# tencent-ailab/pika

Hardware: NVIDIA H100
Metric: utterances/sec RNN-T train step (T=1000,U=150,V=6k) (higher is better)
Workload: dtype bf16

## Files before the change

### include/pika_b200.h

```cpp
#ifndef PIKA_B200_H
#define PIKA_B200_H
#include <stdint.h>

#ifdef __cplusplus
extern "C" {
#endif

#define PK_F32 0
#define PK_BF16 1

const char* pk_last_error(void);
int pk_version(void);
long long pk_launch_count(void);

#define PK_GEMM_MAX_PAIRS 9
#define PK_SEL_ZERO 0
#define PK_SEL_ZB0 1
#define PK_SEL_ZB1 2
#define PK_SEL_KZ 3
#define PK_ACT_NONE 0
#define PK_ACT_RELU 1
#define PK_AUX_NONE 0
#define PK_AUX_ADD 1
#define PK_AUX_MASK_NZ 2
// ... 144 lines not shown
                           const void* dout, long long ld_dout, const float* lse, float* dsum_ws, void* dq, void* dk, void* dv,
                           long long ld_dqkv, int B, int T, int heads, int dh, float alpha, float drop_p, const uint32_t* keep_bits,
                           int chunk_len, int chunk_off, int left_chunks, void* stream);
int pk_attention_chunk_admits_all(int T, int chunk_len, int chunk_off, int left_chunks);
long long pk_colstats_ws_floats(int C);
int pk_bn_fwd(const void* x, void* y, int dtype, long long rows, int C, const float* w, const float* b, float eps,
              int train, float momentum, float* run_mean, float* run_var, float* mean, float* rstd, float* stats_ws,
              void* stream);
int pk_bn_bwd(const void* dy, const void* x, void* dx, int dtype, long long rows, int C, const float* w,
              const float* mean, const float* rstd, int train, int relu_mask, float* dw, float* db, float* ws ,
              void* stream);
int pk_colsum(const void* x, int dtype, long long rows, int C, float* out, float* ws, void* stream);
int pk_layernorm_fwd(const void* x, void* y, int dtype, long long rows, int C, const float* w, const float* b, float eps,
                     float* mean, float* rstd, void* stream);
int pk_layernorm_bwd(const void* dy, const void* x, void* dx, int dtype, long long rows, int C, const float* w,
                     const float* mean, const float* rstd, float* dw, float* db, void* stream);
int pk_softmax_fwd(const float* S, long long ld_s, void* P, void* Pd, int dtype, long long ld_p, long long rows, int n,
                   float drop_p, uint32_t seed, void* stream);
int pk_softmax_masked_fwd(const float* S, long long ld_s, void* P, void* Pd, int dtype, long long ld_p, long long rows, int n,
                          int q_len, int heads, int causal, const uint8_t* key_pad, float drop_p, uint32_t seed, void* stream);
int pk_softmax_chunk_fwd(const float* S, long long ld_s, void* P, void* Pd, int dtype, long long ld_p, long long rows, int n,
                         int chunk_len, int chunk_off, int left_chunks, float drop_p, uint32_t seed, void* stream);
int pk_softmax_bwd(const float* dPd, long long ld_d, const void* P, long long ld_p, void* dS, int dtype, long long rows,
                   int n, float drop_p, uint32_t seed, void* stream);
#define PK_RELPOS_MAX 1024
int pk_softmax_masked_relpos_fwd(const float* S, long long ld_s, const float* QR, long long ld_r, void* P, void* Pd, int dtype,
                                 long long ld_p, long long rows, int n, int q_len, int heads, int causal, const uint8_t* key_pad,
                                 int max_rel, float* Pb, float drop_p, uint32_t seed, void* stream);
int pk_softmax_relpos_bwd(const float* dPd, long long ld_d, const float* G, long long ld_r, const void* P, long long ld_p, void* dS,
                          int dtype, long long rows, int n, int q_len, int heads, int max_rel, float* dSb, float drop_p,
                          uint32_t seed, void* stream);
int pk_dropout(const void* x, void* y, int dtype, long long n, float p, uint32_t seed, void* stream);
int pk_mask_nz(const void* dy, const void* y, void* dx, int dtype, long long n, float scale, void* stream);
int pk_add(const void* a, const void* b, void* o, int dtype, long long n, void* stream);
int pk_log_softmax(const void* x, int dtype, long long ld, float* y, long long rows, int n, float scale, void* stream);
int pk_joint_gate_fwd(const void* ex, const void* py, void* h, int dtype, int B, int T, int U1, int H, int ld_h, void* stream);
int pk_joint_gate_bwd(const void* ex, const void* py, const void* dh, const int* dh_map, void* dex, void* dpy, int dtype, int B, int T,
                      int U1, int H, void* stream);
int pk_lstm_cell_fwd(const float* gx, long long ld_gx, const float* gh, long long ld_gh, const float* c_prev, float* c_out,
                     void* h_out, int dtype, long long ld_h, float* gates_save, int B, int H, void* stream);
int pk_lstm_cell_bwd(const void* dh_out, long long ld_dho, const float* dh_rec, const float* dc_next, const float* gates,
                     const float* c, const float* c_prev, void* dgates, int dtype, float* dc_prev, int B, int H, void* stream);
int pk_embedding_fwd(const long long* idx, const float* table, int E, void* out, int dtype, int ld_out, long long n, void* stream);
int pk_embedding_bwd(const long long* idx, const void* dout, int dtype, int ld, int E, float* dtable, long long n,
                     long long padding_idx, void* stream);

int pk_absmax(const float* x, long long n, float* out, int* nan_flag, void* stream);
int pk_sgd_nesterov_clip(float* p, const float* g, float* buf, long long n, float lr, float momentum, float max_norm,
                         const float* absmax, const int* nan_flag, int first, void* stream);
int pk_bmuf_delta(const float* glob, const float* local, float* delta, long long n, void* stream);
int pk_bmuf_update(float* glob, float* local, float* delta_prev, const float* delta_sum, long long n, int world,
                   float block_momentum, float block_lr, void* stream);
int pk_adam_clip(float* p, const float* g, float* exp_avg, float* exp_avg_sq, float* p_out2, long long n, double lr,
                 double beta1, double beta2, double eps, double bias_correction1, double bias_correction2_sqrt,
                 float max_norm, const float* absmax, const int* nan_flag, void* stream);
int pk_bmuf_adam_update(float* glob, float* local, float* delta_prev, float* exp_avg_g, float* exp_avg_sq_g, float* msg,
                        long long n, int world, double block_momentum, double block_lr, double beta1_tau, double beta1_rho,
                        double beta2_tau, double beta2_rho, void* stream);

long long pk_frontend_workspace_bytes(int B, int n_max, int t_max, int n_mel, int D);
int pk_frontend_fwd(const short* pcm, long long ld_pcm, const int* n_samples, const float* rate, const int* new_len,
                    const float* target_db, const int* n_frames, int B, int n_max, int t_max, int n_mel, int lctx,
                    int rctx, int stride, const float* window, const float* twiddle, const float* mel_w, const int* mel_lo,
                    const int* mel_hi, int frame_len, int frame_shift, int log2_nfft, int snip_edges, int remove_dc,
                    float preemph, int cmn, const float* offset, const float* scale, int f0, int fs,
                    int t0, int ts, void* out, int out_dtype, short* wave_i16_out, void* workspace,
                    long long workspace_bytes, int* err_flag, float dither, unsigned int dither_seed, void* stream);
int pk_fbank(const float* wave, long long ld_wave, const int* n_samples, const int* n_frames, int B, int t_max, int n_mel,
             const float* window, const float* twiddle, const float* mel_w, const int* mel_lo, const int* mel_hi, int frame_len,
             int frame_shift, int log2_nfft, int snip_edges, int remove_dc, float preemph, float* feats, float dither,
             unsigned int dither_seed, void* stream);

long long pk_frontend_noise_rir_workspace_bytes(int B, int n_max, int t_max, int n_mel, int D, int rir_max_len);
int pk_frontend_fwd_noise_rir(const short* pcm, long long ld_pcm, const int* n_samples, const float* rate, const int* new_len,
                              const float* target_db, const int* n_frames, int B, int n_max, int t_max, int n_mel, int lctx,
                              int rctx, int stride, const float* window, const float* twiddle, const float* mel_w,
                              const int* mel_lo, const int* mel_hi, int frame_len, int frame_shift, int log2_nfft, int snip_edges,
                              int remove_dc, float preemph, int cmn, const float* offset, const float* scale, int f0, int fs,
                              int t0, int ts, void* out, int out_dtype, short* wave_i16_out, void* workspace,
                              long long workspace_bytes, int* err_flag, float dither, unsigned int dither_seed, void* stream,
                              const short* noise, const int* noise_idx, const long long* noise_off, const double* snr,
                              const double* noise_rms_db, const short* rir, const long long* rir_off, const int* rir_len,
                              const int* rir_idx, int rir_max_len);

int pk_mfcc(const float* wave, long long ld_wave, const int* n_samples, const int* n_frames, int B, int t_max, int n_mel,
            const float* window, const float* twiddle, const float* mel_w, const int* mel_lo, const int* mel_hi, int frame_len,
            int frame_shift, int log2_nfft, int snip_edges, int remove_dc, float preemph, float* feats, float dither,
            unsigned int dither_seed, void* stream, const float* dct, int num_ceps, int use_energy, int raw_energy,
            float energy_floor, int htk_compat);
int pk_frontend_fwd_mfcc(const short* pcm, long long ld_pcm, const int* n_samples, const float* rate, const int* new_len,
                         const float* target_db, const int* n_frames, int B, int n_max, int t_max, int n_mel, int lctx,
                         int rctx, int stride, const float* window, const float* twiddle, const float* mel_w,
                         const int* mel_lo, const int* mel_hi, int frame_len, int frame_shift, int log2_nfft, int snip_edges,
                         int remove_dc, float preemph, int cmn, const float* offset, const float* scale, int f0, int fs,
                         int t0, int ts, void* out, int out_dtype, short* wave_i16_out, void* workspace,
                         long long workspace_bytes, int* err_flag, float dither, unsigned int dither_seed, void* stream,
                         const short* noise, const int* noise_idx, const long long* noise_off, const double* snr,
                         const double* noise_rms_db, const short* rir, const long long* rir_off, const int* rir_len,
                         const int* rir_idx, int rir_max_len, const float* dct, int num_ceps, int use_energy,
                         int raw_energy, float energy_floor, int htk_compat);

long long pk_conv_same_f64_workspace_bytes(int B, int n_max, int m_max);
int pk_conv_same_f64(const double* x, long long ld_x, const int* n_len, const double* h, long long ld_h, const int* m_len, int B,
                     int n_max, int m_max, double* y, long long ld_y, void* workspace, long long workspace_bytes, void* stream);

int pk_beam_prepare(const int* next_ys, const int* step_ctx, int* t_idx, const void* enc, int dtype, int Tenc, int H, void* enc_hid,
                    const float* embed, int E, void* x_emb, int ld_x, int K, int blk, int rows, void* stream);
int pk_beam_lstm_cell(const float* gates, const int* next_ys, const int* step_ctx, int blk, void* h, int dtype, float* c, int rows, int H,
                      void* stream);
int pk_beam_step_end(int* step_ctx, const int* not_done, int max_steps, void* stream);
int pk_beam_gate(const float* a, void* h, int dtype, int rows, int H, void* stream);
int pk_row_lse(const void* x, int dtype, long long ld, float* lse, long long rows, int n, float scale, void* stream);
int pk_beam_advance(const float* logits, int ldv, const float* row_lse, float sm_scale, const int* t_idx, const int* num_frames, const int* max_len, float* scores,
                    int* next_ys, int* prev_ks, int* hyp_tok, int* hyp_len, float* fin_score, int* fin_step, int* fin_k,
                    int* fin_count, int* eos_top, int* done, int* not_done_total, int B, int K, int V, int L, int cap,
                    const int* step_ctx, int blk, int n_best, int beam_prune, void* stream);
int pk_beam_reorder(const int* prev_ks, const int* step_ctx, const void* h_in, const float* c_in, const int* t_in, void* h_out, float* c_out,
                    int* t_out, int dtype, int K, int H, int layers, int rows, void* stream);
typedef struct {
    const int* arc_off;
    const int* arc_ilabel;
    const double* arc_weight;
    const int* arc_next;
    const double* finals;
    int backoff_id, n_disambig;
    int disambig_ids[4];
} pk_lm_fst;
int pk_beam_advance_lm(const float* logits, int ldv, const float* row_lse, float sm_scale, const int* t_idx, const int* num_frames, const int* max_len, float* scores,
                       int* next_ys, int* prev_ks, int* hyp_tok, int* hyp_len, float* fin_score, int* fin_step, int* fin_k,
                       int* fin_count, int* eos_top, int* done, int* not_done_total, int B, int K, int V, int L, int cap,
                       const int* step_ctx, int blk, int n_best, int beam_prune, const pk_lm_fst* fst, double lm_scale, double nonblk_reward,
                       int* set_state, double* set_cost, int* set_n, float* lm_scores, int max_states, int* err_flag, void* stream);

typedef struct {
    const int* next_ys;
    const int* step_ctx;
    const int* hyp_tok;
    const int* hyp_len;
    int* slot;
    void* pool;
    long long n_entries;
    int blk, rows, S1, layers, D, dtype, init;
} pk_beam_xf_state;
int pk_beam_xf_taps(const pk_beam_xf_state* st, int layer, const float* embed, int E, const void* x_cur, void* taps, int ldc, void* stream);
int pk_beam_xf_attn(const pk_beam_xf_state* st, int layer, const void* qkv, int heads, const float* rel, int max_rel, void* out, void* stream);
int pk_beam_xf_select(const pk_beam_xf_state* st, const void* x, void* h, int H, void* stream);
int pk_beam_xf_slots(const pk_beam_xf_state* st, const int* prev_ks, int K, void* stream);

long long pk_lstm_seq_workspace_bytes(int H);
int pk_lstm_seq_fwd_ex(const float* gx, const void* w_hh_bf16, void* out, int out_dtype, int ldo, float* gates_save, float* cs,
                       const int* lens, int B, int U, int H, int n_dir, int reverse, void* ws, void* stream);
int pk_lstm_seq_bwd_ex(const void* dout, int dtype, int ldo, const float* gates_save, const float* cs, const void* w_hh_bf16,
                       void* dG_bf16, const int* lens, int B, int U, int H, int n_dir, int reverse, void* ws, void* stream);

int pk_gather_rows(const void* src, const int* idx, void* dst, int dtype, long long rows, int C, void* stream);
int pk_scatter_add_rows(const void* src, const int* idx, float* dst, int dtype, long long rows, int C, void* stream);
int pk_ce_grad(const void* z, int dtype, long long ld, const int* tok, const float* coef, float scale, void* dz,
               long long rows, int n, void* stream);

#ifdef __cplusplus
}
#endif
#endif
```

### pika_b200/csrc/lstm_seq.cu

```cuda
#include <cooperative_groups.h>

#include "../../include/pika_b200.h"
#include "common.cuh"

namespace pk {
void count_launch();

constexpr int LS_HJ = 8;
constexpr int LS_MB = 32;
constexpr int LS_THREADS = 256;
constexpr int LS_PAD = 8;

PK_DEVICE void mma_bf16_16816(float (&c)[4], uint32_t a0, uint32_t a1, uint32_t a2, uint32_t a3, uint32_t b0, uint32_t b1) {
    asm volatile(
        "mma.sync.aligned.m16n8k16.row.col.f32.bf16.bf16.f32 {%0,%1,%2,%3}, {%4,%5,%6,%7}, {%8,%9}, {%0,%1,%2,%3};"
        : "+f"(c[0]), "+f"(c[1]), "+f"(c[2]), "+f"(c[3])
        : "r"(a0), "r"(a1), "r"(a2), "r"(a3), "r"(b0), "r"(b1));
}
PK_DEVICE uint4 ldcg16(const void* p) {
    uint4 r;
    asm volatile("ld.global.cg.v4.u32 {%0,%1,%2,%3}, [%4];" : "=r"(r.x), "=r"(r.y), "=r"(r.z), "=r"(r.w) : "l"(p));
    return r;
}
PK_DEVICE void bulk_g2s(void* smem_dst, const void* gsrc, uint32_t bytes, uint64_t* bar) {
    asm volatile("cp.async.bulk.shared::cluster.global.mbarrier::complete_tx::bytes [%0], [%1], %2, [%3];" ::"r"(smem_u32(smem_dst)),
                 "l"(gsrc), "r"(bytes), "r"(smem_u32(bar))
                 : "memory");
}
PK_DEVICE void bulk_g2s_mc(void* smem_dst, const void* gsrc, uint32_t bytes, uint64_t* bar, uint16_t mask) {
    asm volatile("cp.async.bulk.shared::cluster.global.mbarrier::complete_tx::bytes.multicast::cluster [%0], [%1], %2, [%3], %4;" ::"r"(
                     smem_u32(smem_dst)),
                 "l"(gsrc), "r"(bytes), "r"(smem_u32(bar)), "h"(mask)
                 : "memory");
}
PK_DEVICE void fence_proxy_async_all() { asm volatile("fence.proxy.async;" ::: "memory"); }

PK_DEVICE void grid_barrier(unsigned int* counter, unsigned int step_index, unsigned int nct) {
    const unsigned int target = nct * step_index;
    __syncthreads();
    if (threadIdx.x == 0) {
        asm volatile("red.release.gpu.global.add.u32 [%0], 1;" ::"l"(counter) : "memory");
        unsigned int seen;
        do {
            asm volatile("ld.acquire.gpu.global.u32 %0, [%1];" : "=r"(seen) : "l"(counter) : "memory");
        } while (seen < target);
    }
    __syncthreads();
}
PK_DEVICE float sigm(float x) { return 1.f / (1.f + __expf(-x)); }

PK_DEVICE void load_lens(const int* lens, int B, int U, int* len_s, int* steps_s) {
    if (threadIdx.x < 32) {
        int L = 0;
        if ((int)threadIdx.x < B) L = lens ? min(max(lens[threadIdx.x], 0), U) : U;
        len_s[threadIdx.x] = L;
        int m = L;
#pragma unroll
        for (int o = 16; o > 0; o >>= 1) m = max(m, __shfl_xor_sync(0xffffffffu, m, o));
        if (threadIdx.x == 0) *steps_s = m;
    }
}

struct LsDir {
    int d;
    bool rev;
    int j0;
    unsigned nct;
};
PK_DEVICE LsDir ls_dir(int H, int reverse) {
    LsDir r;
    r.nct = (unsigned)(H / LS_HJ);
    r.d = (int)(blockIdx.x / r.nct);
    r.rev = gridDim.x > r.nct ? r.d == 1 : reverse != 0;
    r.j0 = (int)(blockIdx.x - r.d * r.nct) * LS_HJ;
    return r;
}

template <typename T>
__global__ void __launch_bounds__(LS_THREADS, 1) lstm_seq_fwd_kernel(const float* __restrict__ gx, const __nv_bfloat16* __restrict__ w_hh,
                                                                     T* __restrict__ out, int ldo, __nv_bfloat16* hx, float* __restrict__ gates_save,
                                                                     float* __restrict__ cs, const int* __restrict__ lens, int B, int Bt, int U,
                                                                     int H, int reverse, unsigned int* counter) {
    extern __shared__ __align__(16) uint8_t sm_raw[];
    const int P = H + LS_PAD;
    __nv_bfloat16* w_s = reinterpret_cast<__nv_bfloat16*>(sm_raw);
    __nv_bfloat16* h_s = w_s + 32 * P;
    float* g_s = reinterpret_cast<float*>(h_s + 32 * P);
    const int tid = threadIdx.x, warp = tid >> 5, lane = tid & 31;
    const LsDir dir = ls_dir(H, reverse);
    const int j0 = dir.j0;
    gx += (long long)dir.d * Bt * U * 4 * H;
    w_hh += (long long)dir.d * 4 * H * H;
    out += dir.d * H;
    hx += (long long)dir.d * 2 * LS_MB * H;
    gates_save += (long long)dir.d * U * Bt * 4 * H;
    cs += (long long)dir.d * U * Bt * H;
    counter += dir.d * 32;
    __shared__ int len_s[LS_MB], steps_s;
    load_lens(lens, B, U, len_s, &steps_s);
    const int vec_per_row = H / 8;
    for (int i = tid; i < 32 * vec_per_row; i += LS_THREADS) {
        const int r = i / vec_per_row, v = i - r * vec_per_row;
        const int grow = (r >> 3) * H + j0 + (r & 7);
        *reinterpret_cast<uint4*>(w_s + r * P + v * 8) = *reinterpret_cast<const uint4*>(w_hh + (long long)grow * H + v * 8);
    }
    const int cb = tid >> 3, cj = tid & 7;
    float c_state = 0.f;
    const int mt = warp & 1, nt = warp >> 1;
    const int g = lane >> 2, tq = lane & 3;
    __shared__ __align__(8) uint64_t h_bar;
    if (tid == 0) { mbar_init(&h_bar, 1); mbar_fence_init(); }
    uint32_t h_phase = 0;
    const uint32_t cn = cluster_nctarank(), cr = cluster_ctarank();
    const uint16_t cmask = (uint16_t)((1u << cn) - 1u);
    __syncthreads();
    if (cn > 1) cluster_sync_all();
    const int S = steps_s, L = len_s[cb];
    for (int s = 0; s < S; ++s) {
        const bool active = s < L;
        const int t = dir.rev ? L - 1 - s : s;
        float acc[4] = {0.f, 0.f, 0.f, 0.f};
        float gx_i = 0.f, gx_f = 0.f, gx_g = 0.f, gx_o = 0.f;
        if (active) {
            const float* gxr = gx + ((long long)cb * U + t) * 4 * H + j0 + cj;
            gx_i = __ldg(gxr); gx_f = __ldg(gxr + H); gx_g = __ldg(gxr + 2 * H); gx_o = __ldg(gxr + 3 * H);
        }
        if (s > 0) {
            const __nv_bfloat16* src = hx + (long long)((s - 1) & 1) * LS_MB * H;
            if (warp == 0) {
                fence_proxy_async_all();
                if (lane == 0) mbar_arrive_expect_tx(&h_bar, 32u * (uint32_t)H * 2u);
                __syncwarp();
                if (cn == 1) bulk_g2s(h_s + lane * P, src + (long long)lane * H, (uint32_t)H * 2u, &h_bar);
                else if ((lane % cn) == cr) bulk_g2s_mc(h_s + lane * P, src + (long long)lane * H, (uint32_t)H * 2u, &h_bar, cmask);
            }
            mbar_wait(&h_bar, h_phase);
            h_phase ^= 1;
            const __nv_bfloat16* ar0 = h_s + (mt * 16 + g) * P + 2 * tq;
            const __nv_bfloat16* ar1 = ar0 + 8 * P;
            const __nv_bfloat16* br = w_s + (nt * 8 + g) * P + 2 * tq;
            float acc1[4] = {0.f, 0.f, 0.f, 0.f}, acc2[4] = {0.f, 0.f, 0.f, 0.f}, acc3[4] = {0.f, 0.f, 0.f, 0.f};
            auto mma_at = [&](float (&c)[4], int k0) {
                const uint32_t a0 = *reinterpret_cast<const uint32_t*>(ar0 + k0), a1 = *reinterpret_cast<const uint32_t*>(ar1 + k0);
                const uint32_t a2 = *reinterpret_cast<const uint32_t*>(ar0 + k0 + 8), a3 = *reinterpret_cast<const uint32_t*>(ar1 + k0 + 8);
                const uint32_t b0 = *reinterpret_cast<const uint32_t*>(br + k0), b1 = *reinterpret_cast<const uint32_t*>(br + k0 + 8);
                mma_bf16_16816(c, a0, a1, a2, a3, b0, b1);
            };
#pragma unroll 4
            for (int k0 = 0; k0 < H; k0 += 64) {
                mma_at(acc, k0);
                mma_at(acc1, k0 + 16);
                mma_at(acc2, k0 + 32);
                mma_at(acc3, k0 + 48);
            }
#pragma unroll
            for (int e = 0; e < 4; ++e) acc[e] = (acc[e] + acc1[e]) + (acc2[e] + acc3[e]);
        }
        g_s[(mt * 16 + g) * 33 + nt * 8 + 2 * tq] = acc[0];
        g_s[(mt * 16 + g) * 33 + nt * 8 + 2 * tq + 1] = acc[1];
        g_s[(mt * 16 + g + 8) * 33 + nt * 8 + 2 * tq] = acc[2];
        g_s[(mt * 16 + g + 8) * 33 + nt * 8 + 2 * tq + 1] = acc[3];
        __syncthreads();
        if (active) {
            const float gi = sigm(g_s[cb * 33 + cj] + gx_i);
            const float gf = sigm(g_s[cb * 33 + 8 + cj] + gx_f);
            const float gg = tanhf(g_s[cb * 33 + 16 + cj] + gx_g);
            const float go = sigm(g_s[cb * 33 + 24 + cj] + gx_o);
            c_state = gf * c_state + gi * gg;
            const float hv = go * tanhf(c_state);
            out[((long long)cb * U + t) * ldo + j0 + cj] = from_f32<T>(hv);
            hx[(long long)(s & 1) * LS_MB * H + (long long)cb * H + j0 + cj] = __float2bfloat16_rn(hv);
            float* gs = gates_save + ((long long)t * Bt + cb) * 4 * H + j0 + cj;
            gs[0] = gi; gs[H] = gf; gs[2 * H] = gg; gs[3 * H] = go;
            cs[((long long)t * Bt + cb) * H + j0 + cj] = c_state;
        } else {
            hx[(long long)(s & 1) * LS_MB * H + (long long)cb * H + j0 + cj] = __float2bfloat16_rn(0.f);
            if (cb < B) out[((long long)cb * U + s) * ldo + j0 + cj] = from_f32<T>(0.f);
        }
        if (s + 1 < S) grid_barrier(counter, (unsigned int)(s + 1), dir.nct);
    }
    if (cb < B)
        for (int t = S; t < U; ++t) out[((long long)cb * U + t) * ldo + j0 + cj] = from_f32<T>(0.f);
}

template <typename T>
__global__ void __launch_bounds__(LS_THREADS, 1) lstm_seq_bwd_kernel(const T* __restrict__ dout, int ldo, const float* __restrict__ gates_save,
                                                                     const float* __restrict__ cs, const __nv_bfloat16* __restrict__ w_hh,
                                                                     __nv_bfloat16* dG, const __nv_bfloat16* zrow, const int* __restrict__ lens,
                                                                     int B, int Bt, int U, int H, int reverse, unsigned int* counter) {
    extern __shared__ __align__(16) uint8_t sm_raw[];
    const int G4 = 4 * H;
    const int PW = G4 + LS_PAD;
    const int KQ = G4 / 4;
    const int PD = KQ + LS_PAD;
    __nv_bfloat16* wt_s = reinterpret_cast<__nv_bfloat16*>(sm_raw);
    __nv_bfloat16* d_s = wt_s + LS_HJ * PW;
    float* r_s = reinterpret_cast<float*>(d_s + 2 * 32 * PD);
    __shared__ __align__(8) uint64_t q_bar[2];
    const int tid = threadIdx.x, warp = tid >> 5, lane = tid & 31;
    const LsDir dir = ls_dir(H, reverse);
    const int j0 = dir.j0;
    dout += dir.d * H;
    gates_save += (long long)dir.d * U * Bt * G4;
    cs += (long long)dir.d * U * Bt * H;
    w_hh += (long long)dir.d * G4 * H;
    dG += (long long)dir.d * U * Bt * G4;
    counter += dir.d * 32;
    __shared__ int len_s[LS_MB], steps_s;
    load_lens(lens, B, U, len_s, &steps_s);
    for (int i = tid; i < G4 * LS_HJ; i += LS_THREADS) {
        const int r = i / LS_HJ, jj = i - r * LS_HJ;
        wt_s[jj * PW + r] = w_hh[(long long)r * H + j0 + jj];
    }
    for (int i = tid; i < 2 * 32 * PD / 8; i += LS_THREADS) reinterpret_cast<uint4*>(d_s)[i] = make_uint4(0, 0, 0, 0);
    for (int i = tid; i < 4 * 32 * 9; i += LS_THREADS) r_s[i] = 0.f;
    if (tid == 0) { mbar_init(&q_bar[0], 1); mbar_init(&q_bar[1], 1); mbar_fence_init(); }
    const int cb = tid >> 3, cj = tid & 7;
    float dc_state = 0.f;
    const int mt = warp & 1, kg = warp >> 1;
    const int g = lane >> 2, tq = lane & 3;
    uint32_t q_phase[2] = {0, 0};
    const uint32_t cn = cluster_nctarank(), cr = cluster_ctarank();
    const uint16_t cmask = (uint16_t)((1u << cn) - 1u);
    __syncthreads();
    if (cn > 1) cluster_sync_all();
    const int S = steps_s, L = len_s[cb];
    if (cb < B)
        for (int t = S; t < U; ++t) {
            __nv_bfloat16* d = dG + ((long long)t * Bt + cb) * G4 + j0 + cj;
            d[0] = d[H] = d[2 * H] = d[3 * H] = __float2bfloat16_rn(0.f);
        }
    const int Lr = len_s[lane];
    for (int s = S - 1; s >= 0; --s) {
        const bool active = s < L;
        const int t = dir.rev ? L - 1 - s : s;
        float pgi = 0.f, pgf = 0.f, pgg = 0.f, pgo = 0.f, pc = 0.f, pcp = 0.f, pdo = 0.f;
        if (active) {
            const int j = j0 + cj;
            const int tp = dir.rev ? t + 1 : t - 1;
            const float* gs = gates_save + ((long long)t * Bt + cb) * G4 + j;
            pgi = __ldg(gs); pgf = __ldg(gs + H); pgg = __ldg(gs + 2 * H); pgo = __ldg(gs + 3 * H);
            pc = __ldg(cs + ((long long)t * Bt + cb) * H + j);
            pcp = s > 0 ? __ldg(cs + ((long long)tp * Bt + cb) * H + j) : 0.f;
            pdo = to_f32<T>(dout[((long long)cb * U + t) * ldo + j]);
        }
        if (s < S - 1) {
            const int tn = dir.rev ? Lr - 2 - s : s + 1;
            const __nv_bfloat16* src = s + 1 < Lr ? dG + ((long long)tn * Bt + lane) * G4 : zrow;
            auto issue = [&](int qtr) {
                if (warp == 0) {
                    fence_proxy_async_all();
                    if (lane == 0) mbar_arrive_expect_tx(&q_bar[qtr & 1], (uint32_t)B * (uint32_t)KQ * 2u);
                    __syncwarp();
                    __nv_bfloat16* dst = d_s + ((qtr & 1) * 32 + lane) * PD;
                    const __nv_bfloat16* from = src + qtr * KQ;
                    if (lane < B) {
                        if (cn == 1) bulk_g2s(dst, from, (uint32_t)KQ * 2u, &q_bar[qtr & 1]);
                        else if ((lane % cn) == cr) bulk_g2s_mc(dst, from, (uint32_t)KQ * 2u, &q_bar[qtr & 1], cmask);
                    }
                }
            };
            issue(0);
            issue(1);
            float acc[4] = {0.f, 0.f, 0.f, 0.f}, accb[4] = {0.f, 0.f, 0.f, 0.f}, accc[4] = {0.f, 0.f, 0.f, 0.f}, accd[4] = {0.f, 0.f, 0.f, 0.f};
            const int kspan = KQ / 4;
            for (int qtr = 0; qtr < 4; ++qtr) {
                mbar_wait(&q_bar[qtr & 1], q_phase[qtr & 1]);
                q_phase[qtr & 1] ^= 1;
                const __nv_bfloat16* ar0 = d_s + ((qtr & 1) * 32 + mt * 16 + g) * PD + kg * kspan + 2 * tq;
                const __nv_bfloat16* ar1 = ar0 + 8 * PD;
                const __nv_bfloat16* br = wt_s + g * PW + qtr * KQ + kg * kspan + 2 * tq;
                auto mma_at = [&](float (&c)[4], int k0) {
                    const uint32_t a0 = *reinterpret_cast<const uint32_t*>(ar0 + k0), a1 = *reinterpret_cast<const uint32_t*>(ar1 + k0);
                    const uint32_t a2 = *reinterpret_cast<const uint32_t*>(ar0 + k0 + 8), a3 = *reinterpret_cast<const uint32_t*>(ar1 + k0 + 8);
                    const uint32_t b0 = *reinterpret_cast<const uint32_t*>(br + k0), b1 = *reinterpret_cast<const uint32_t*>(br + k0 + 8);
                    mma_bf16_16816(c, a0, a1, a2, a3, b0, b1);
                };
                int k0 = 0;
#pragma unroll 4
                for (; k0 + 64 <= kspan; k0 += 64) {
                    mma_at(acc, k0);
                    mma_at(accb, k0 + 16);
                    mma_at(accc, k0 + 32);
                    mma_at(accd, k0 + 48);
                }
                for (; k0 < kspan; k0 += 16) mma_at(acc, k0);
                if (qtr + 2 < 4) {
                    if (cn == 1) __syncthreads();
                    else cluster_sync_all();
                    issue(qtr + 2);
                }
            }
#pragma unroll
            for (int e = 0; e < 4; ++e) acc[e] = (acc[e] + accb[e]) + (accc[e] + accd[e]);
            float* r_k = r_s + kg * 32 * 9;
            r_k[(mt * 16 + g) * 9 + 2 * tq] = acc[0];
            r_k[(mt * 16 + g) * 9 + 2 * tq + 1] = acc[1];
            r_k[(mt * 16 + g + 8) * 9 + 2 * tq] = acc[2];
            r_k[(mt * 16 + g + 8) * 9 + 2 * tq + 1] = acc[3];
        }
        __syncthreads();
        if (active) {
            const int j = j0 + cj;
            const float gi = pgi, gf = pgf, gg = pgg, go = pgo, c = pc, cp = pcp;
            const float* r_c = r_s + cb * 9 + cj;
            const float dh = pdo + (((r_c[0] + r_c[32 * 9]) + r_c[2 * 32 * 9]) + r_c[3 * 32 * 9]);
            const float tc = tanhf(c);
            const float dc = dh * go * (1.f - tc * tc) + dc_state;
            __nv_bfloat16* d = dG + ((long long)t * Bt + cb) * G4 + j;
            d[0] = __float2bfloat16_rn(dc * gg * gi * (1.f - gi));
            d[H] = __float2bfloat16_rn(dc * cp * gf * (1.f - gf));
            d[2 * H] = __float2bfloat16_rn(dc * gi * (1.f - gg * gg));
            d[3 * H] = __float2bfloat16_rn(dh * tc * go * (1.f - go));
            dc_state = dc * gf;
        } else if (cb < B) {
            __nv_bfloat16* d = dG + ((long long)s * Bt + cb) * G4 + j0 + cj;
            d[0] = d[H] = d[2 * H] = d[3 * H] = __float2bfloat16_rn(0.f);
        }
        if (s > 0) grid_barrier(counter, (unsigned int)(S - s), dir.nct);
    }
}
}

using namespace pk;

static int lstm_launch(const void* fn, int grid, int smem, void** args, cudaStream_t st, int* cluster_cache) {
    cudaLaunchConfig_t cfg = {};
    cfg.gridDim = dim3(grid); cfg.blockDim = dim3(LS_THREADS); cfg.dynamicSmemBytes = smem; cfg.stream = st;
    cudaLaunchAttribute attr[2];
    attr[0].id = cudaLaunchAttributeCooperative; attr[0].val.cooperative = 1;
    if (*cluster_cache == 0) {
        int pick = 1;
        for (int cs = 8; cs >= 2; cs >>= 1) {
            if (grid % cs) continue;
            attr[1].id = cudaLaunchAttributeClusterDimension; attr[1].val.clusterDim.x = cs; attr[1].val.clusterDim.y = 1; attr[1].val.clusterDim.z = 1;
            cfg.attrs = attr; cfg.numAttrs = 2;
            int ncl = 0;
            if (cudaOccupancyMaxActiveClusters(&ncl, fn, &cfg) == cudaSuccess && ncl * cs >= grid) { pick = cs; break; }
            (void)cudaGetLastError();
        }
        *cluster_cache = pick;
    }
    attr[1].id = cudaLaunchAttributeClusterDimension; attr[1].val.clusterDim.x = *cluster_cache; attr[1].val.clusterDim.y = 1; attr[1].val.clusterDim.z = 1;
    cfg.attrs = attr; cfg.numAttrs = 2;
    PK_CHECK_CUDA(cudaLaunchKernelExC(&cfg, fn, args));
    return 0;
}
static inline bool aligned16(const void* p) { return (reinterpret_cast<uintptr_t>(p) & 15) == 0; }
static int lstm_seq_check(int B, int U, int H, int n_dir, int ldo) {
    PK_CHECK_ARG(B >= 1, "empty batch");
    PK_CHECK_ARG(U >= 1, "U must be >= 1");
    PK_CHECK_ARG(n_dir == 1 || n_dir == 2, "n_dir must be 1 or 2");
    PK_CHECK_ARG(H >= 64 && H % 64 == 0 && n_dir * H / LS_HJ <= num_sms(), "H must be a multiple of 64 with n_dir * H/8 <= #SMs");
    PK_CHECK_ARG(ldo >= n_dir * H, "ldo must be >= n_dir * H");
    return 0;
}
static int* lstm_cluster_slot(int (*cache)[2][64], int fl, int n_dir, int H) { return &cache[fl][n_dir - 1][(H / 64) & 63]; }

extern "C" long long pk_lstm_seq_workspace_bytes(int H) { return 2ll * LS_MB * H * 2 + 256 + 4ll * H * 2; }

extern "C" int pk_lstm_seq_fwd_ex(const float* gx, const void* w_hh_bf16, void* out, int out_dtype, int ldo, float* gates_save, float* cs,
                                  const int* lens, int B, int U, int H, int n_dir, int reverse, void* ws, void* stream) {
    int rc = lstm_seq_check(B, U, H, n_dir, ldo);
    if (rc) return rc;
    PK_CHECK_ARG(aligned16(w_hh_bf16) && aligned16(ws), "pk_lstm_seq_fwd_ex: w_hh, ws must be 16-byte aligned");
    cudaStream_t st = reinterpret_cast<cudaStream_t>(stream);
    unsigned int* counter = reinterpret_cast<unsigned int*>(ws);
    __nv_bfloat16* hx = reinterpret_cast<__nv_bfloat16*>(reinterpret_cast<unsigned char*>(ws) + 256);
    const int smem = 2 * 32 * (H + LS_PAD) * 2 + 32 * 33 * 4;
    const __nv_bfloat16* w = reinterpret_cast<const __nv_bfloat16*>(w_hh_bf16);
    const void* fn = out_dtype == PK_BF16 ? (const void*)lstm_seq_fwd_kernel<__nv_bfloat16> : (const void*)lstm_seq_fwd_kernel<float>;
    PK_CHECK_CUDA(cudaFuncSetAttribute(fn, cudaFuncAttributeMaxDynamicSharedMemorySize, smem));
    const size_t es = out_dtype == PK_BF16 ? 2 : 4;
    const int grid = n_dir * H / LS_HJ;
    static int cluster_f[2][2][64] = {};
    for (int b0 = 0; b0 < B; b0 += LS_MB) {
        int nb = B - b0 < LS_MB ? B - b0 : LS_MB, Bt = B;
        const float* gx_c = gx + (long long)b0 * U * 4 * H;
        void* out_c = reinterpret_cast<unsigned char*>(out) + (size_t)b0 * U * ldo * es;
        float* gs_c = gates_save + (long long)b0 * 4 * H;
        float* cs_c = cs + (long long)b0 * H;
        const int* lens_c = lens ? lens + b0 : nullptr;
        PK_CHECK_CUDA(cudaMemsetAsync(counter, 0, 256, st));
        void* args[] = {(void*)&gx_c, (void*)&w, (void*)&out_c, (void*)&ldo, (void*)&hx, (void*)&gs_c, (void*)&cs_c, (void*)&lens_c, (void*)&nb,
                        (void*)&Bt, (void*)&U, (void*)&H, (void*)&reverse, (void*)&counter};
        rc = lstm_launch(fn, grid, smem, args, st, lstm_cluster_slot(cluster_f, out_dtype == PK_BF16 ? 0 : 1, n_dir, H));
        if (rc) return rc;
        count_launch();
    }
    return 0;
}
extern "C" int pk_lstm_seq_bwd_ex(const void* dout, int dtype, int ldo, const float* gates_save, const float* cs, const void* w_hh_bf16,
                                  void* dG_bf16, const int* lens, int B, int U, int H, int n_dir, int reverse, void* ws, void* stream) {
    int rc = lstm_seq_check(B, U, H, n_dir, ldo);
    if (rc) return rc;
    PK_CHECK_ARG(aligned16(dG_bf16) && aligned16(ws), "pk_lstm_seq_bwd_ex: dG, ws must be 16-byte aligned");
    cudaStream_t st = reinterpret_cast<cudaStream_t>(stream);
    unsigned int* counter = reinterpret_cast<unsigned int*>(ws);
    const __nv_bfloat16* zrow = reinterpret_cast<const __nv_bfloat16*>(reinterpret_cast<unsigned char*>(ws) + 256 + 2ll * LS_MB * n_dir * H * 2);
    const int G4 = 4 * H;
    const int smem = LS_HJ * (G4 + LS_PAD) * 2 + 2 * 32 * (G4 / 4 + LS_PAD) * 2 + 4 * 32 * 9 * 4;
    const __nv_bfloat16* w = reinterpret_cast<const __nv_bfloat16*>(w_hh_bf16);
    const void* fn = dtype == PK_BF16 ? (const void*)lstm_seq_bwd_kernel<__nv_bfloat16> : (const void*)lstm_seq_bwd_kernel<float>;
    PK_CHECK_CUDA(cudaFuncSetAttribute(fn, cudaFuncAttributeMaxDynamicSharedMemorySize, smem));
    const size_t es = dtype == PK_BF16 ? 2 : 4;
    const int grid = n_dir * H / LS_HJ;
    static int cluster_b[2][2][64] = {};
    for (int b0 = 0; b0 < B; b0 += LS_MB) {
        int nb = B - b0 < LS_MB ? B - b0 : LS_MB, Bt = B;
        const void* dout_c = reinterpret_cast<const unsigned char*>(dout) + (size_t)b0 * U * ldo * es;
        const float* gs_c = gates_save + (long long)b0 * G4;
        const float* cs_c = cs + (long long)b0 * H;
        __nv_bfloat16* dg = reinterpret_cast<__nv_bfloat16*>(dG_bf16) + (long long)b0 * G4;
        const int* lens_c = lens ? lens + b0 : nullptr;
        PK_CHECK_CUDA(cudaMemsetAsync(counter, 0, 256, st));
        void* args[] = {(void*)&dout_c, (void*)&ldo, (void*)&gs_c, (void*)&cs_c, (void*)&w, (void*)&dg, (void*)&zrow, (void*)&lens_c, (void*)&nb,
                        (void*)&Bt, (void*)&U, (void*)&H, (void*)&reverse, (void*)&counter};
        rc = lstm_launch(fn, grid, smem, args, st, lstm_cluster_slot(cluster_b, dtype == PK_BF16 ? 0 : 1, n_dir, H));
        if (rc) return rc;
        count_launch();
    }
    return 0;
}
```

Baseline: 285.6.

## Split LSTM backward recurrence K dimension across cluster CTAs with DSMEM reduction

The backward LSTM recurrence kernel is templated on cluster size. Each CTA in a cluster now holds only a K-slice of W_hh^T for all the cluster's hidden columns and multiplies it against its own K-slice of dG. Partial sums are exchanged through distributed shared memory with a cluster barrier, which replaces the multicast TMA of full dG rows and the per-CTA full-K GEMV. The aim is to cut per-step smem load and TMA traffic on the sequential critical path. The price is extra cluster syncs, DSMEM reads and more complex launch selection, and a force-cluster override API is added.

```diff
diff --git a/include/pika_b200.h b/include/pika_b200.h
--- a/include/pika_b200.h
+++ b/include/pika_b200.h
@@ -320,6 +320,7 @@
                        const int* lens, int B, int U, int H, int n_dir, int reverse, void* ws, void* stream);
 int pk_lstm_seq_bwd_ex(const void* dout, int dtype, int ldo, const float* gates_save, const float* cs, const void* w_hh_bf16,
                        void* dG_bf16, const int* lens, int B, int U, int H, int n_dir, int reverse, void* ws, void* stream);
+int pk_lstm_seq_force_cluster(int cs);
 
 int pk_gather_rows(const void* src, const int* idx, void* dst, int dtype, long long rows, int C, void* stream);
 int pk_scatter_add_rows(const void* src, const int* idx, float* dst, int dtype, long long rows, int C, void* stream);
diff --git a/pika_b200/csrc/lstm_seq.cu b/pika_b200/csrc/lstm_seq.cu
--- a/pika_b200/csrc/lstm_seq.cu
+++ b/pika_b200/csrc/lstm_seq.cu
@@ -74,6 +74,25 @@
     r.rev = gridDim.x > r.nct ? r.d == 1 : reverse != 0;
     r.j0 = (int)(blockIdx.x - r.d * r.nct) * LS_HJ;
     return r;
+}
+
+PK_DEVICE uint32_t dsmem_map(const void* p, uint32_t rank) {
+    uint32_t r;
+    asm volatile("mapa.shared::cluster.u32 %0, %1, %2;" : "=r"(r) : "r"(smem_u32(p)), "r"(rank));
+    return r;
+}
+PK_DEVICE float ld_dsmem(uint32_t addr) {
+    float v;
+    asm volatile("ld.shared::cluster.f32 %0, [%1];" : "=f"(v) : "r"(addr) : "memory");
+    return v;
+}
+template <int N> PK_DEVICE float tree_sum(const float* v) {
+    if constexpr (N == 1) return v[0];
+    else return tree_sum<N / 2>(v) + tree_sum<N / 2>(v + N / 2);
+}
+template <int CS> PK_DEVICE void ls_cluster_sync() {
+    if constexpr (CS > 1) cluster_sync_all();
+    else __syncthreads();
 }
 
 template <typename T>
@@ -183,23 +202,39 @@
         for (int t = S; t < U; ++t) out[((long long)cb * U + t) * ldo + j0 + cj] = from_f32<T>(0.f);
 }
 
-template <typename T>
+template <int CS> struct LsBwdGeom {
+    static constexpr int NKG = 8 / CS;
+    static constexpr int NQ = CS == 1 ? 4 : 1;
+    static constexpr int NB = CS == 1 ? 2 : 1;
+    static constexpr int NRB = CS == 1 ? 1 : 2;
+    static constexpr int PR = 8 * CS + 8;
+};
+static int ls_bwd_smem(int H, int CS) {
+    const int ks = 4 * H / CS, nq = CS == 1 ? 4 : 1, nb = CS == 1 ? 2 : 1, nrb = CS == 1 ? 1 : 2;
+    return LS_HJ * CS * (ks + LS_PAD) * 2 + nb * 32 * (ks / nq + LS_PAD) * 2 + nrb * (8 / CS) * 32 * (8 * CS + 8) * 4;
+}
+
+template <typename T, int CS>
 __global__ void __launch_bounds__(LS_THREADS, 1) lstm_seq_bwd_kernel(const T* __restrict__ dout, int ldo, const float* __restrict__ gates_save,
                                                                      const float* __restrict__ cs, const __nv_bfloat16* __restrict__ w_hh,
                                                                      __nv_bfloat16* dG, const __nv_bfloat16* zrow, const int* __restrict__ lens,
                                                                      int B, int Bt, int U, int H, int reverse, unsigned int* counter) {
+    using Gm = LsBwdGeom<CS>;
     extern __shared__ __align__(16) uint8_t sm_raw[];
     const int G4 = 4 * H;
-    const int PW = G4 + LS_PAD;
-    const int KQ = G4 / 4;
-    const int PD = KQ + LS_PAD;
+    const int KS = G4 / CS;
+    const int nq = Gm::NQ;
+    const int KC = KS / nq;
+    const int PW = KS + LS_PAD, PD = KC + LS_PAD;
     __nv_bfloat16* wt_s = reinterpret_cast<__nv_bfloat16*>(sm_raw);
-    __nv_bfloat16* d_s = wt_s + LS_HJ * PW;
-    float* r_s = reinterpret_cast<float*>(d_s + 2 * 32 * PD);
-    __shared__ __align__(8) uint64_t q_bar[2];
+    __nv_bfloat16* d_s = wt_s + LS_HJ * CS * PW;
+    float* r_s = reinterpret_cast<float*>(d_s + Gm::NB * 32 * PD);
+    __shared__ __align__(8) uint64_t q_bar[Gm::NB];
     const int tid = threadIdx.x, warp = tid >> 5, lane = tid & 31;
     const LsDir dir = ls_dir(H, reverse);
     const int j0 = dir.j0;
+    const uint32_t cr = CS > 1 ? cluster_ctarank() : 0;
+    const int jc0 = j0 - (int)cr * LS_HJ, kb = (int)cr * KS;
     dout += dir.d * H;
     gates_save += (long long)dir.d * U * Bt * G4;
     cs += (long long)dir.d * U * Bt * H;
@@ -208,22 +243,24 @@
     counter += dir.d * 32;
     __shared__ int len_s[LS_MB], steps_s;
     load_lens(lens, B, U, len_s, &steps_s);
-    for (int i = tid; i < G4 * LS_HJ; i += LS_THREADS) {
-        const int r = i / LS_HJ, jj = i - r * LS_HJ;
-        wt_s[jj * PW + r] = w_hh[(long long)r * H + j0 + jj];
-    }
-    for (int i = tid; i < 2 * 32 * PD / 8; i += LS_THREADS) reinterpret_cast<uint4*>(d_s)[i] = make_uint4(0, 0, 0, 0);
-    for (int i = tid; i < 4 * 32 * 9; i += LS_THREADS) r_s[i] = 0.f;
-    if (tid == 0) { mbar_init(&q_bar[0], 1); mbar_init(&q_bar[1], 1); mbar_fence_init(); }
+    for (int i = tid; i < KS * LS_HJ * CS; i += LS_THREADS) {
+        const int r = i / (LS_HJ * CS), n = i - r * (LS_HJ * CS);
+        wt_s[n * PW + r] = w_hh[(long long)(kb + r) * H + jc0 + n];
+    }
+    for (int i = tid; i < Gm::NB * 32 * PD / 8; i += LS_THREADS) reinterpret_cast<uint4*>(d_s)[i] = make_uint4(0, 0, 0, 0);
+    if (tid == 0) {
+        for (int i = 0; i < Gm::NB; ++i) mbar_init(&q_bar[i], 1);
+        mbar_fence_init();
+    }
     const int cb = tid >> 3, cj = tid & 7;
     float dc_state = 0.f;
-    const int mt = warp & 1, kg = warp >> 1;
+    const int nt = warp % CS, kg = warp / CS;
     const int g = lane >> 2, tq = lane & 3;
-    uint32_t q_phase[2] = {0, 0};
-    const uint32_t cn = cluster_nctarank(), cr = cluster_ctarank();
-    const uint16_t cmask = (uint16_t)((1u << cn) - 1u);
+    uint32_t q_phase[Gm::NB] = {};
+    uint32_t peer[CS];
+#pragma unroll
+    for (int p = 0; p < CS; ++p) peer[p] = CS > 1 ? dsmem_map(r_s, (uint32_t)p) : smem_u32(r_s);
     __syncthreads();
-    if (cn > 1) cluster_sync_all();
     const int S = steps_s, L = len_s[cb];
     if (cb < B)
         for (int t = S; t < U; ++t) {
@@ -244,67 +281,77 @@
             pcp = s > 0 ? __ldg(cs + ((long long)tp * Bt + cb) * H + j) : 0.f;
             pdo = to_f32<T>(dout[((long long)cb * U + t) * ldo + j]);
         }
+        float rec = 0.f;
         if (s < S - 1) {
             const int tn = dir.rev ? Lr - 2 - s : s + 1;
-            const __nv_bfloat16* src = s + 1 < Lr ? dG + ((long long)tn * Bt + lane) * G4 : zrow;
-            auto issue = [&](int qtr) {
+            const __nv_bfloat16* src = (s + 1 < Lr ? dG + ((long long)tn * Bt + lane) * G4 : zrow) + kb;
+            auto issue = [&](int q) {
                 if (warp == 0) {
+                    uint64_t* bar = &q_bar[q % Gm::NB];
                     fence_proxy_async_all();
-                    if (lane == 0) mbar_arrive_expect_tx(&q_bar[qtr & 1], (uint32_t)B * (uint32_t)KQ * 2u);
+                    if (lane == 0) mbar_arrive_expect_tx(bar, (uint32_t)B * (uint32_t)KC * 2u);
                     __syncwarp();
-                    __nv_bfloat16* dst = d_s + ((qtr & 1) * 32 + lane) * PD;
-                    const __nv_bfloat16* from = src + qtr * KQ;
-                    if (lane < B) {
-                        if (cn == 1) bulk_g2s(dst, from, (uint32_t)KQ * 2u, &q_bar[qtr & 1]);
-                        else if ((lane % cn) == cr) bulk_g2s_mc(dst, from, (uint32_t)KQ * 2u, &q_bar[qtr & 1], cmask);
-                    }
+                    if (lane < B) bulk_g2s(d_s + ((q % Gm::NB) * 32 + lane) * PD, src + q * KC, (uint32_t)KC * 2u, bar);
                 }
             };
-            issue(0);
-            issue(1);
-            float acc[4] = {0.f, 0.f, 0.f, 0.f}, accb[4] = {0.f, 0.f, 0.f, 0.f}, accc[4] = {0.f, 0.f, 0.f, 0.f}, accd[4] = {0.f, 0.f, 0.f, 0.f};
-            const int kspan = KQ / 4;
-            for (int qtr = 0; qtr < 4; ++qtr) {
-                mbar_wait(&q_bar[qtr & 1], q_phase[qtr & 1]);
-                q_phase[qtr & 1] ^= 1;
-                const __nv_bfloat16* ar0 = d_s + ((qtr & 1) * 32 + mt * 16 + g) * PD + kg * kspan + 2 * tq;
-                const __nv_bfloat16* ar1 = ar0 + 8 * PD;
-                const __nv_bfloat16* br = wt_s + g * PW + qtr * KQ + kg * kspan + 2 * tq;
-                auto mma_at = [&](float (&c)[4], int k0) {
-                    const uint32_t a0 = *reinterpret_cast<const uint32_t*>(ar0 + k0), a1 = *reinterpret_cast<const uint32_t*>(ar1 + k0);
-                    const uint32_t a2 = *reinterpret_cast<const uint32_t*>(ar0 + k0 + 8), a3 = *reinterpret_cast<const uint32_t*>(ar1 + k0 + 8);
-                    const uint32_t b0 = *reinterpret_cast<const uint32_t*>(br + k0), b1 = *reinterpret_cast<const uint32_t*>(br + k0 + 8);
-                    mma_bf16_16816(c, a0, a1, a2, a3, b0, b1);
+#pragma unroll
+            for (int q = 0; q < Gm::NB; ++q)
+                if (q < nq) issue(q);
+            float acc[2][2][4] = {};
+            const int nks = KC / 16;
+#pragma unroll
+            for (int q = 0; q < Gm::NQ; ++q) {
+                if (q >= nq) break;
+                mbar_wait(&q_bar[q % Gm::NB], q_phase[q % Gm::NB]);
+                q_phase[q % Gm::NB] ^= 1;
+                const __nv_bfloat16* ar = d_s + ((q % Gm::NB) * 32 + g) * PD + 2 * tq;
+                const __nv_bfloat16* br = wt_s + (nt * 8 + g) * PW + q * KC + 2 * tq;
+                auto mma_at = [&](float (&c)[2][4], int ks) {
+                    const int k = ks * 16;
+                    const uint32_t b0 = *reinterpret_cast<const uint32_t*>(br + k), b1 = *reinterpret_cast<const uint32_t*>(br + k + 8);
+#pragma unroll
+                    for (int mt = 0; mt < 2; ++mt) {
+                        const __nv_bfloat16* r0 = ar + mt * 16 * PD + k;
+                        mma_bf16_16816(c[mt], *reinterpret_cast<const uint32_t*>(r0), *reinterpret_cast<const uint32_t*>(r0 + 8 * PD),
+                                       *reinterpret_cast<const uint32_t*>(r0 + 8), *reinterpret_cast<const uint32_t*>(r0 + 8 * PD + 8), b0, b1);
+                    }
                 };
-                int k0 = 0;
+                int ks = kg;
 #pragma unroll 4
-                for (; k0 + 64 <= kspan; k0 += 64) {
-                    mma_at(acc, k0);
-                    mma_at(accb, k0 + 16);
-                    mma_at(accc, k0 + 32);
-                    mma_at(accd, k0 + 48);
+                for (; ks + Gm::NKG < nks; ks += 2 * Gm::NKG) {
+                    mma_at(acc[0], ks);
+                    mma_at(acc[1], ks + Gm::NKG);
                 }
-                for (; k0 < kspan; k0 += 16) mma_at(acc, k0);
-                if (qtr + 2 < 4) {
-                    if (cn == 1) __syncthreads();
-                    else cluster_sync_all();
-                    issue(qtr + 2);
+                if (ks < nks) mma_at(acc[0], ks);
+                if (q + Gm::NB < nq) {
+                    __syncthreads();
+                    issue(q + Gm::NB);
                 }
             }
-#pragma unroll
-            for (int e = 0; e < 4; ++e) acc[e] = (acc[e] + accb[e]) + (accc[e] + accd[e]);
-            float* r_k = r_s + kg * 32 * 9;
-            r_k[(mt * 16 + g) * 9 + 2 * tq] = acc[0];
-            r_k[(mt * 16 + g) * 9 + 2 * tq + 1] = acc[1];
-            r_k[(mt * 16 + g + 8) * 9 + 2 * tq] = acc[2];
-            r_k[(mt * 16 + g + 8) * 9 + 2 * tq + 1] = acc[3];
-        }
-        __syncthreads();
+            float* rw = r_s + (((Gm::NRB == 2 ? (s & 1) : 0) * Gm::NKG + kg) * 32) * Gm::PR;
+#pragma unroll
+            for (int mt = 0; mt < 2; ++mt) {
+                float* o = rw + (mt * 16 + g) * Gm::PR + nt * 8 + 2 * tq;
+                *reinterpret_cast<float2*>(o) = make_float2(acc[0][mt][0] + acc[1][mt][0], acc[0][mt][1] + acc[1][mt][1]);
+                *reinterpret_cast<float2*>(o + 8 * Gm::PR) = make_float2(acc[0][mt][2] + acc[1][mt][2], acc[0][mt][3] + acc[1][mt][3]);
+            }
+            ls_cluster_sync<CS>();
+            const uint32_t off = (uint32_t)((((Gm::NRB == 2 ? (s & 1) : 0) * Gm::NKG) * 32 + cb) * Gm::PR + (int)cr * 8 + cj) * 4u;
+            float part[8];
+#pragma unroll
+            for (int p = 0; p < CS; ++p)
+#pragma unroll
+                for (int k = 0; k < Gm::NKG; ++k) {
+                    const uint32_t a = peer[p] + off + (uint32_t)(k * 32 * Gm::PR * 4);
+                    if constexpr (CS > 1) part[p * Gm::NKG + k] = ld_dsmem(a);
+                    else part[p * Gm::NKG + k] = *reinterpret_cast<const float*>(reinterpret_cast<const uint8_t*>(r_s) + (a - peer[0]));
+                }
+            rec = tree_sum<8>(part);
+        }
         if (active) {
             const int j = j0 + cj;
             const float gi = pgi, gf = pgf, gg = pgg, go = pgo, c = pc, cp = pcp;
-            const float* r_c = r_s + cb * 9 + cj;
-            const float dh = pdo + (((r_c[0] + r_c[32 * 9]) + r_c[2 * 32 * 9]) + r_c[3 * 32 * 9]);
+            const float dh = pdo + rec;
             const float tc = tanhf(c);
             const float dc = dh * go * (1.f - tc * tc) + dc_state;
             __nv_bfloat16* d = dG + ((long long)t * Bt + cb) * G4 + j;
@@ -319,31 +366,48 @@
         }
         if (s > 0) grid_barrier(counter, (unsigned int)(S - s), dir.nct);
     }
+    if constexpr (CS > 1) cluster_sync_all();
 }
 }
 
 using namespace pk;
 
-static int lstm_launch(const void* fn, int grid, int smem, void** args, cudaStream_t st, int* cluster_cache) {
+static int g_lstm_force_cluster = 0;
+
+static int lstm_launch(const void* const fn[4], const int smem[4], int grid, void** args, cudaStream_t st, int* cluster_cache) {
     cudaLaunchConfig_t cfg = {};
-    cfg.gridDim = dim3(grid); cfg.blockDim = dim3(LS_THREADS); cfg.dynamicSmemBytes = smem; cfg.stream = st;
+    cfg.gridDim = dim3(grid); cfg.blockDim = dim3(LS_THREADS); cfg.stream = st;
     cudaLaunchAttribute attr[2];
     attr[0].id = cudaLaunchAttributeCooperative; attr[0].val.cooperative = 1;
-    if (*cluster_cache == 0) {
-        int pick = 1;
-        for (int cs = 8; cs >= 2; cs >>= 1) {
-            if (grid % cs) continue;
-            attr[1].id = cudaLaunchAttributeClusterDimension; attr[1].val.clusterDim.x = cs; attr[1].val.clusterDim.y = 1; attr[1].val.clusterDim.z = 1;
-            cfg.attrs = attr; cfg.numAttrs = 2;
-            int ncl = 0;
-            if (cudaOccupancyMaxActiveClusters(&ncl, fn, &cfg) == cudaSuccess && ncl * cs >= grid) { pick = cs; break; }
-            (void)cudaGetLastError();
-        }
-        *cluster_cache = pick;
-    }
-    attr[1].id = cudaLaunchAttributeClusterDimension; attr[1].val.clusterDim.x = *cluster_cache; attr[1].val.clusterDim.y = 1; attr[1].val.clusterDim.z = 1;
-    cfg.attrs = attr; cfg.numAttrs = 2;
-    PK_CHECK_CUDA(cudaLaunchKernelExC(&cfg, fn, args));
+    auto set_cluster = [&](int cs) {
+        attr[1].id = cudaLaunchAttributeClusterDimension; attr[1].val.clusterDim.x = cs; attr[1].val.clusterDim.y = 1; attr[1].val.clusterDim.z = 1;
+        cfg.attrs = attr; cfg.numAttrs = 2;
+    };
+    auto lg = [](int cs) { return cs == 8 ? 3 : cs == 4 ? 2 : cs == 2 ? 1 : 0; };
+    int pick = g_lstm_force_cluster;
+    if (!pick) {
+        if (*cluster_cache == 0) {
+            int best = 1;
+            for (int cs = 8; cs >= 2; cs >>= 1) {
+                const int i = lg(cs);
+                if (grid % cs || smem[i] > 227 * 1024) continue;
+                PK_CHECK_CUDA(cudaFuncSetAttribute(fn[i], cudaFuncAttributeMaxDynamicSharedMemorySize, smem[i]));
+                cfg.dynamicSmemBytes = smem[i];
+                set_cluster(cs);
+                int ncl = 0;
+                if (cudaOccupancyMaxActiveClusters(&ncl, fn[i], &cfg) == cudaSuccess && ncl * cs >= grid) { best = cs; break; }
+                (void)cudaGetLastError();
+            }
+            *cluster_cache = best;
+        }
+        pick = *cluster_cache;
+    }
+    const int i = lg(pick);
+    PK_CHECK_ARG(smem[i] <= 227 * 1024, "pk_lstm_seq: shared memory of the recurrence exceeds 227 KB");
+    PK_CHECK_CUDA(cudaFuncSetAttribute(fn[i], cudaFuncAttributeMaxDynamicSharedMemorySize, smem[i]));
+    cfg.dynamicSmemBytes = smem[i];
+    set_cluster(pick);
+    PK_CHECK_CUDA(cudaLaunchKernelExC(&cfg, fn[i], args));
     return 0;
 }
 static inline bool aligned16(const void* p) { return (reinterpret_cast<uintptr_t>(p) & 15) == 0; }
@@ -357,6 +421,13 @@
 }
 static int* lstm_cluster_slot(int (*cache)[2][64], int fl, int n_dir, int H) { return &cache[fl][n_dir - 1][(H / 64) & 63]; }
 
+extern "C" int pk_lstm_seq_force_cluster(int cs) {
+    PK_CHECK_ARG(cs == 0 || cs == 1 || cs == 2 || cs == 4 || cs == 8, "pk_lstm_seq_force_cluster: cs must be 0, 1, 2, 4 or 8");
+    const int prev = g_lstm_force_cluster;
+    g_lstm_force_cluster = cs;
+    return prev;
+}
+
 extern "C" long long pk_lstm_seq_workspace_bytes(int H) { return 2ll * LS_MB * H * 2 + 256 + 4ll * H * 2; }
 
 extern "C" int pk_lstm_seq_fwd_ex(const float* gx, const void* w_hh_bf16, void* out, int out_dtype, int ldo, float* gates_save, float* cs,
@@ -367,11 +438,13 @@
     cudaStream_t st = reinterpret_cast<cudaStream_t>(stream);
     unsigned int* counter = reinterpret_cast<unsigned int*>(ws);
     __nv_bfloat16* hx = reinterpret_cast<__nv_bfloat16*>(reinterpret_cast<unsigned char*>(ws) + 256);
-    const int smem = 2 * 32 * (H + LS_PAD) * 2 + 32 * 33 * 4;
     const __nv_bfloat16* w = reinterpret_cast<const __nv_bfloat16*>(w_hh_bf16);
-    const void* fn = out_dtype == PK_BF16 ? (const void*)lstm_seq_fwd_kernel<__nv_bfloat16> : (const void*)lstm_seq_fwd_kernel<float>;
-    PK_CHECK_CUDA(cudaFuncSetAttribute(fn, cudaFuncAttributeMaxDynamicSharedMemorySize, smem));
-    const size_t es = out_dtype == PK_BF16 ? 2 : 4;
+    const bool bf = out_dtype == PK_BF16;
+    const void* f = bf ? (const void*)lstm_seq_fwd_kernel<__nv_bfloat16> : (const void*)lstm_seq_fwd_kernel<float>;
+    const void* fn[4] = {f, f, f, f};
+    const int sm = 2 * 32 * (H + LS_PAD) * 2 + 32 * 33 * 4;
+    const int smem[4] = {sm, sm, sm, sm};
+    const size_t es = bf ? 2 : 4;
     const int grid = n_dir * H / LS_HJ;
     static int cluster_f[2][2][64] = {};
     for (int b0 = 0; b0 < B; b0 += LS_MB) {
@@ -384,7 +457,7 @@
         PK_CHECK_CUDA(cudaMemsetAsync(counter, 0, 256, st));
         void* args[] = {(void*)&gx_c, (void*)&w, (void*)&out_c, (void*)&ldo, (void*)&hx, (void*)&gs_c, (void*)&cs_c, (void*)&lens_c, (void*)&nb,
                         (void*)&Bt, (void*)&U, (void*)&H, (void*)&reverse, (void*)&counter};
-        rc = lstm_launch(fn, grid, smem, args, st, lstm_cluster_slot(cluster_f, out_dtype == PK_BF16 ? 0 : 1, n_dir, H));
+        rc = lstm_launch(fn, smem, grid, args, st, lstm_cluster_slot(cluster_f, bf ? 0 : 1, n_dir, H));
         if (rc) return rc;
         count_launch();
     }
@@ -399,11 +472,14 @@
     unsigned int* counter = reinterpret_cast<unsigned int*>(ws);
     const __nv_bfloat16* zrow = reinterpret_cast<const __nv_bfloat16*>(reinterpret_cast<unsigned char*>(ws) + 256 + 2ll * LS_MB * n_dir * H * 2);
     const int G4 = 4 * H;
-    const int smem = LS_HJ * (G4 + LS_PAD) * 2 + 2 * 32 * (G4 / 4 + LS_PAD) * 2 + 4 * 32 * 9 * 4;
     const __nv_bfloat16* w = reinterpret_cast<const __nv_bfloat16*>(w_hh_bf16);
-    const void* fn = dtype == PK_BF16 ? (const void*)lstm_seq_bwd_kernel<__nv_bfloat16> : (const void*)lstm_seq_bwd_kernel<float>;
-    PK_CHECK_CUDA(cudaFuncSetAttribute(fn, cudaFuncAttributeMaxDynamicSharedMemorySize, smem));
-    const size_t es = dtype == PK_BF16 ? 2 : 4;
+    const bool bf = dtype == PK_BF16;
+    const void* fn[4] = {bf ? (const void*)lstm_seq_bwd_kernel<__nv_bfloat16, 1> : (const void*)lstm_seq_bwd_kernel<float, 1>,
+                         bf ? (const void*)lstm_seq_bwd_kernel<__nv_bfloat16, 2> : (const void*)lstm_seq_bwd_kernel<float, 2>,
+                         bf ? (const void*)lstm_seq_bwd_kernel<__nv_bfloat16, 4> : (const void*)lstm_seq_bwd_kernel<float, 4>,
+                         bf ? (const void*)lstm_seq_bwd_kernel<__nv_bfloat16, 8> : (const void*)lstm_seq_bwd_kernel<float, 8>};
+    const int smem[4] = {ls_bwd_smem(H, 1), ls_bwd_smem(H, 2), ls_bwd_smem(H, 4), ls_bwd_smem(H, 8)};
+    const size_t es = bf ? 2 : 4;
     const int grid = n_dir * H / LS_HJ;
     static int cluster_b[2][2][64] = {};
     for (int b0 = 0; b0 < B; b0 += LS_MB) {
@@ -416,7 +492,7 @@
         PK_CHECK_CUDA(cudaMemsetAsync(counter, 0, 256, st));
         void* args[] = {(void*)&dout_c, (void*)&ldo, (void*)&gs_c, (void*)&cs_c, (void*)&w, (void*)&dg, (void*)&zrow, (void*)&lens_c, (void*)&nb,
                         (void*)&Bt, (void*)&U, (void*)&H, (void*)&reverse, (void*)&counter};
-        rc = lstm_launch(fn, grid, smem, args, st, lstm_cluster_slot(cluster_b, dtype == PK_BF16 ? 0 : 1, n_dir, H));
+        rc = lstm_launch(fn, smem, grid, args, st, lstm_cluster_slot(cluster_b, bf ? 0 : 1, n_dir, H));
         if (rc) return rc;
         count_launch();
     }
```

Measured after the change: 286.5 (median of 6 runs). No clear change (+0.3%).
